# justinkay/aldi

Measured on AMD Instinct MI355X. Metric: images/sec (student+teacher ALDI step), R50-FPN 1333x800, higher is better.
Workload: dtype bf16

## Files before the change

### aldi_amd/csrc/host.h

```cpp
#pragma once
#include "../../include/aldi_hip.h"

int aldi_set_error_msg(int code, const char* msg);

typedef uint16_t bf16_t;

#define ALDI_KNOBS(X) \
    X(igemm_xcd, 1) X(igemm_tile, 0) X(igemm_dbg, 0) X(igemm_bigtile_min, 1024) X(igemm_bigtile, 64) X(igemm_bigtile_k, 768) X(igemm_lintile_min, 768) \
    X(igemm_halo, 1) X(igemm_force, 0) X(igemm_k64_min, 1024) X(igemm_group, 1) X(igemm_narrow_k, 512) X(igemm_splitk_tile, 2) X(igemm_halo_f32, 0) \
    X(igemm_f32_tile64_max, 4096) X(igemm_direct, 15) X(igemm_lean, 1) X(igemm_halo64_mid, 0) X(igemm_ws, 1) X(igemm_ws_wgs, 512) X(igemm_ws_min, 40000) \
    X(wgrad_lean, 1) X(wgrad_big_min, 28) X(wgrad_big_slots, 256) X(wgrad_slots, 384) X(wgrad_xcd, 1) \
    X(igemm_halo_ilv, 1) X(igemm_halo_small, 0) X(igemm_halo96, 0) \
    X(wgrad_dma, 0) X(wgrad_dbg, 0) X(wgrad_group_slots, 0) X(wgrad_group_epi, 24) X(wgrad_db, 0) X(wgrad_ordered, 1) X(wgrad_big_group, 1) X(wgrad_big_epi, 12) \
    X(wgrad_big_group_min, 64) X(wgrad_lds_pad_kb, 0) X(wgrad_f32_tile128, 1) X(wgrad_dma64, 3) X(wgrad_ilv, 0) \
    X(msda_gather, 7) X(msda_gather_list, 1500) X(msda_bin, 1) X(msda_bin_list, 512) X(roialign_sep, 1) X(roialign_bwd_rows, 2) \
    X(colsum_blocks, 256) X(colsum_minrows, 16) X(colsum_nt, 1024) X(colsum_block_kb, 384) \
    X(stem_mfma, 1) X(stem_pool_wgs, 0) X(sab_blocks, 512) X(ln_bwd_blocks, 512) X(ln_bwd_blocks_narrow, 1024) X(rpn_topk_fused, 1) X(ema_blocks, 2048) X(nms_mask_tri, 1) X(match_wave, 1)

struct AldiTuning {
#define ALDI_KNOB_FIELD(name, dflt) int name;
    ALDI_KNOBS(ALDI_KNOB_FIELD)
#undef ALDI_KNOB_FIELD
};
AldiTuning& aldi_tuning();
void aldi_note_dispatch(const char* kernel);

static inline int cdiv(long a, long b) { return (int)((a + b - 1) / b); }
```

### aldi_amd/csrc/roi.hip

```cpp
#include "common.h"
#include "loss_rows.h"
#include "sortscan.h"
#include "nms.h"
#include <hip/amd_detail/amd_hip_unsafe_atomics.h>


namespace {

__global__ void roi_append_gt_kernel(const float4* __restrict__ props, const int* __restrict__ pcount, int P,
                                     const float4* __restrict__ gt, const int* __restrict__ gcount, int Gmax,
                                     float4* __restrict__ cand, int* __restrict__ ccount, int Pcap) {
    const int n = blockIdx.y;
    const int i = blockIdx.x * blockDim.x + threadIdx.x;
    const int pc = pcount[n], gc = gcount[n];
    if (i == 0) ccount[n] = pc + gc;
    if (i >= Pcap) return;
    float4 v = make_float4(0, 0, 0, 0);
    if (i < pc) v = props[(long)n * P + i];
    else if (i < pc + gc) v = gt[(long)n * Gmax + (i - pc)];
    cand[(long)n * Pcap + i] = v;
}

__global__ void roi_classes_kernel(const int* __restrict__ labels, const int* __restrict__ best_idx, const int* __restrict__ gt_classes,
                                   const int* __restrict__ gcount, int Gmax, int L, int K, int* __restrict__ cls) {
// ... 827 lines not shown
        }
    }
#pragma unroll
    for (int r = 0; r < 2; ++r) {
        const int py = py0 + r;
        if (py >= H || px0 + px >= W) continue;
        const long o = (((long)b * H + py) * W + px0 + px) * C + cg * 4;
        if constexpr (sizeof(GT) == 2) {
            bf16_t* G = reinterpret_cast<bf16_t*>(ft.g[l]) + o;
#pragma unroll
            for (int j = 0; j < 8; ++j) {
                uint2 v;
                v.x = pack2_bf16(acc[r][j].x, acc[r][j].y); v.y = pack2_bf16(acc[r][j].z, acc[r][j].w);
                *reinterpret_cast<uint2*>(G + j * 32) = v;
            }
        } else {
            float* G = ft.g[l] + o;
#pragma unroll
            for (int j = 0; j < 8; ++j) *reinterpret_cast<float4*>(G + j * 32) = acc[r][j];
        }
    }
}

__global__ __launch_bounds__(256) void box_loss_kernel(const float* __restrict__ pred, int Cp, int K, int R,
                                                       const float* __restrict__ rois, const int* __restrict__ cls, const float4* __restrict__ gtb,
                                                       float wx, float wy, float ww, float wh, float gs_cls, float gs_box,
                                                       float* __restrict__ grad, float* __restrict__ loss ) {
    __shared__ float red[16];
    const int r = blockIdx.x * blockDim.x + threadIdx.x;
    float l_cls = 0.f, l_box = 0.f;
    const float invR = 1.f / (float)max(R, 1);
    if (r < R)
        box_loss_row(pred + (long)r * Cp, K, cls[r], rois + (long)r * 5, gtb[r], wx, wy, ww, wh, invR, gs_cls, gs_box, grad ? grad + (long)r * Cp : nullptr,
                     l_cls, l_box);
    float s0 = block_sum(l_cls, red);
    float s1 = block_sum(l_box, red);
    if (threadIdx.x == 0) {
        if (s0 != 0.f) unsafeAtomicAdd(loss + 0, s0 * invR);
        if (s1 != 0.f) unsafeAtomicAdd(loss + 1, s1 * invR);
    }
}

constexpr int kMaxLossChunks = 8;
struct BoxLossChunk {
    int r0, r1, blk0;
    float gs_cls, gs_box;
// ... 209 lines not shown
    GatherGeom gg;
    gg.N = N;
    const int rows = dtype == ALDI_BF16 && aldi_tuning().roialign_bwd_rows != 1 ? 2 : 1;
    int off = 0;
    for (int l = 0; l < 4; ++l) {
        if (!ft.g[l]) return aldi_set_error_msg(ALDI_ERR_ARG, "roialign_backward: missing gradient map");
        gg.blk_off[l] = off;
        gg.segs[l] = cdiv(ft.W[l], kSeg);
        off += N * cdiv(ft.H[l], rows) * gg.segs[l];
    }
    gg.blk_off[4] = off;
    hipStream_t st = static_cast<hipStream_t>(stream);
    if (rows == 2 && grad_dtype == ALDI_BF16)
        hipLaunchKernelGGL((roialign_bwd_gather2_kernel<bf16_t>), dim3(off), dim3(256), 0, st, ft, gg, rois, R, P, (const bf16_t*)g_pooled, rois_sorted);
    else if (rows == 2)
        hipLaunchKernelGGL((roialign_bwd_gather2_kernel<float>), dim3(off), dim3(256), 0, st, ft, gg, rois, R, P, (const bf16_t*)g_pooled, rois_sorted);
    else if (dtype == ALDI_BF16 && grad_dtype == ALDI_BF16)
        hipLaunchKernelGGL((roialign_bwd_gather_kernel<bf16_t, bf16_t>), dim3(off), dim3(256), 0, st, ft, gg, rois, R, P, (const bf16_t*)g_pooled, rois_sorted);
    else if (dtype == ALDI_BF16)
        hipLaunchKernelGGL((roialign_bwd_gather_kernel<bf16_t, float>), dim3(off), dim3(256), 0, st, ft, gg, rois, R, P, (const bf16_t*)g_pooled, rois_sorted);
    else if (dtype == ALDI_F32)
        hipLaunchKernelGGL((roialign_bwd_gather_kernel<float, float>), dim3(off), dim3(256), 0, st, ft, gg, rois, R, P, (const float*)g_pooled, rois_sorted);
    else return aldi_set_error_msg(ALDI_ERR_ARG, "roialign_backward: bad dtype");
    ALDI_CHECK_LAUNCH();
    return ALDI_OK;
}

extern "C" int aldi_box_loss(const float* pred, int Cp, int K, int R, const float* rois, const int* cls, const float* gt_boxes,
                             const float* weights4, float grad_scale_cls, float grad_scale_box, float* grad, float* loss2, aldi_stream_t stream) {
    if (!pred || !rois || !cls || !gt_boxes || !loss2 || !weights4) return aldi_set_error_msg(ALDI_ERR_ARG, "box_loss: null pointer");
    if (R <= 0) return ALDI_OK;
    hipLaunchKernelGGL(box_loss_kernel, dim3(cdiv(R, 256)), dim3(256), 0, static_cast<hipStream_t>(stream), pred, Cp, K, R, rois, cls, (const float4*)gt_boxes,
                       weights4[0], weights4[1], weights4[2], weights4[3], grad_scale_cls, grad_scale_box, grad, loss2);
    ALDI_CHECK_LAUNCH();
    return ALDI_OK;
}

extern "C" int aldi_box_losses_fused(const float* pred, int Cp, int K, const float* rois, const int* cls, const float* gt_boxes, const float* weights4,
                                     const aldi_box_loss_chunk* chunks, int nchunks, float* grad, void* grad_lo, aldi_stream_t stream) {
    if (!pred || !rois || !cls || !gt_boxes || !weights4 || !chunks || !grad) return aldi_set_error_msg(ALDI_ERR_ARG, "box_losses_fused: null pointer");
    if (nchunks < 1 || nchunks > kMaxLossChunks || (Cp & 1)) return aldi_set_error_msg(ALDI_ERR_ARG, "box_losses_fused: 1 .. 8 chunks, even row length");
    BoxLossArgs A;
    A.n = 0;
    int blk = 0;
    for (int i = 0; i < nchunks; ++i) {
        const aldi_box_loss_chunk& q = chunks[i];
// ... 63 lines not shown
```

### aldi_amd/engine.py

```python
from __future__ import annotations

import contextlib
import dataclasses
import inspect
import math
import os
from collections import OrderedDict
from typing import Dict, List, Optional, Sequence, Tuple

import torch

from . import ops
from .arch import FC_DIM, FPN_C, NUM_ANCHORS, POOL, STAGE_BLOCKS, Packed, ParamLayout, pad_to

PIXEL_MEAN = (103.530, 116.280, 123.675)
PIXEL_STD = (1.0, 1.0, 1.0)
ANCHOR_SIZES = (32, 64, 128, 256, 512)
ANCHOR_RATIOS = (0.5, 1.0, 2.0)
STRIDES = (4, 8, 16, 32, 64)
GMAX = 128
RPN_BATCH, RPN_POS_FRAC = 256, 0.5
ROI_BATCH, ROI_POS_FRAC = 512, 0.25
RPN_PRE = (2000, 1000)
RPN_POST = (1000, 1000)
RPN_NMS = 0.7
ROI_WEIGHTS = (10.0, 10.0, 5.0, 5.0)
SCORE_THRESH, NMS_TEST, DETS = 0.05, 0.5, 100


_FAST_RANDPERM = None


def randperm_prefix(n: int, k: int) -> torch.Tensor:
    global _FAST_RANDPERM
    from . import _lib as L
# ... 299 lines not shown
    if code & 1:
        raise FloatingPointError(f"{who}: predicted boxes or scores contain Inf/NaN. Training has diverged.")
    if code & 2:
        raise RuntimeError(f"{who}: sparse RPN-head backward: more active pixels than (2 * BATCH_SIZE_PER_IMAGE + 4 * positives) per image; "
                           "the excess was dropped, gradients of this step are wrong -- or, from the detection post-processing: a row of class "
                           "scores contains Inf/NaN; the row was dropped")
    if code & 4:
        raise RuntimeError(f"{who}: detection post-processing: more than 8192 candidates above SCORE_THRESH_TEST in one image; the excess was dropped")
    if code & 8:
        raise RuntimeError(f"{who}: RPN top-k: the group barrier of `topk_fused_kernel` timed out (its workgroups were not co-resident); the candidates "
                           "of this step are wrong.  Set ALDI_RPN_TOPK_FUSED=0 for the five-launch path")
    if code:
        raise RuntimeError(f"{who}: device error word {code}")


class Ctx(dict):
    __getattr__ = dict.__getitem__
    __setattr__ = dict.__setitem__


class RCNN:
    p = D2Params()
    stats_sink = None

    def __init__(self, weights: Weights, num_classes: int, params: Optional[D2Params] = None):
        self.wts = weights
        if params is not None:
            self.p = params
        self.K = num_classes
        self.device, self.dtype = weights.device, weights.dtype
        self.Cp = weights.layout.t["box_pred"].rows
        self.Ch = weights.layout.t["rpn_head_out"].rows
        self._anchor_cache: Dict[tuple, tuple] = {}
        self._ws: Dict[str, torch.Tensor] = {}
        self.err = torch.zeros(1, dtype=torch.int32, device=self.device)
        torch.set_num_threads(1)
        idx = lambda n: int(n.rsplit(".", 1)[1])
        names = list(getattr(weights.layout, "t", {}))
        self.img_da_layers = sorted((n for n in names if n.startswith("img_align.model.")), key=idx)
        self.ins_da_layers = sorted((n for n in names if n.startswith("ins_align.model.")), key=idx)
        self.has_img_da, self.has_ins_da = bool(self.img_da_layers), bool(self.ins_da_layers)
        self.fused_stem = os.environ.get("ALDI_FUSED_STEM", "1") == "1"
        self.wgrad_tail_split = int(os.environ.get("ALDI_WGRAD_TAIL_SPLIT", "2"))
        self.group_wgrad = os.environ.get("ALDI_WGRAD_GROUP", "1") == "1"
        self.mask_bits = os.environ.get("ALDI_MASK_BITS", "1") == "1"
        self.mask_bits_inner = os.environ.get("ALDI_MASK_BITS_INNER", "1") == "1"
        self.level_groups = os.environ.get("ALDI_LEVEL_GROUPS", "1") == "1"
        self.fused_res2 = os.environ.get("ALDI_FUSED_RES2", "1") == "1"
        self.fused_res2_shortcut = os.environ.get("ALDI_FUSED_RES2_SHORTCUT", "1") == "1"
        self.fused_stage_entrance = os.environ.get("ALDI_FUSED_STAGE_ENTRANCE", "1") == "1"
        self._wg_queue: list = []
        self.sparse_rpn_backward = os.environ.get("ALDI_RPN_SPARSE_BWD", "1") == "1"
        spec = getattr(weights.layout, "img_da", None)
        self.img_da_level = ("p2", "p3", "p4", "p5", "p6").index(spec["layer"]) if spec else 0

    def stage_images(self, images: Sequence[torch.Tensor]):
        sizes = [(int(im.shape[1]), int(im.shape[2])) for im in images]
        Hs = pad_to(max(s[0] for s in sizes), 32)
        Ws = pad_to(max(s[1] for s in sizes), 32)
        N = len(images)
        if all(im.is_cuda for im in images):
            st = torch.zeros((N, 3, Hs, Ws), dtype=torch.uint8, device=self.device)
            for i, im in enumerate(images):
                st[i, :, : sizes[i][0], : sizes[i][1]] = im
        else:
            host = torch.zeros((N, 3, Hs, Ws), dtype=torch.uint8).pin_memory()
            for i, im in enumerate(images):
                host[i, :, : sizes[i][0], : sizes[i][1]] = im
            st = host.to(self.device, non_blocking=True)
        hw = torch.tensor(sizes, dtype=torch.int32).to(self.device)
        return st, sizes, hw

    def stage_gt(self, instances: Sequence[dict]):
        N = len(instances)
        gb = torch.zeros((N, GMAX, 4), dtype=torch.float32)
# ... 584 lines not shown
        else:
            scratch = torch.empty((N, GMAX), dtype=torch.int32, device=dev)
            ops.roi_prepare(props, prop_count, P, gt["boxes"], gt["classes"], gt["count"], GMAX, N, self.K, self.p.roi_iou, cand, ccount, best_iou, best_idx,
                            scratch, labels, cls)
            ops.compact_labels(cls, Lc, N, self.K, lists, counts)
        return dict(cand=cand, cls=cls, best_idx=best_idx, lists=lists, counts=counts, Lc=Lc, counts_tail=cbuf)

    def _roi_gather(self, c: Ctx, prep: dict, sel, nsel, nsel_h, gt, N, row_off_dev=None):
        dev = self.device
        rows = [a + b for a, b in nsel_h]
        row_off = [0]
        for r in rows[:-1]:
            row_off.append(row_off[-1] + r)
        R = sum(rows)
        c.R, c.rows = R, rows
        c.rois = torch.empty((max(R, 1), 5), dtype=torch.float32, device=dev)
        c.r_cls = torch.empty((max(R, 1),), dtype=torch.int32, device=dev)
        c.r_gt = torch.empty((max(R, 1), 4), dtype=torch.float32, device=dev)
        c.r_idx = torch.empty((max(R, 1),), dtype=torch.int32, device=dev)
        if row_off_dev is None:
            row_off_dev = torch.tensor(row_off, dtype=torch.int32).to(dev)
        ops.roi_gather(prep["cand"], prep["cls"], prep["best_idx"], prep["Lc"], prep["lists"], sel, nsel, self.p.roi_batch,
                       row_off_dev, gt["boxes"], gt["count"], GMAX, N, c.rois, c.r_cls, c.r_gt, c.r_idx)

    def roi_sample(self, c: Ctx, props, prop_count, gt, N):
        prep = self._roi_prepare(props, prop_count, gt, N)
        host_counts = prep["counts"].cpu().tolist()
        c.roi_host_counts = host_counts
        sel, nsel, nsel_h = self._sample(host_counts, self.p.roi_batch, self.p.roi_pos_frac)
        self._roi_gather(c, prep, sel, nsel, nsel_h, gt, N)

    def roi_forward(self, c: Ctx):
        R = c.R
        pooled = torch.empty((R, POOL, POOL, FPN_C), dtype=self.dtype, device=self.device)
        ops.roialign(self.roi_feats(c), c.rois, R, POOL, pooled, backward=False)
        c.pred, _ = self.box_head(pooled, c)

    def box_head_on(self, c_feats: Ctx, rois: torch.Tensor, R: int):
        pooled = torch.empty((R, POOL, POOL, FPN_C), dtype=self.dtype, device=self.device)
        ops.roialign(self.roi_feats(c_feats), rois, R, POOL, pooled, backward=False)
        pred, fc2 = self.box_head(pooled)
        return pred

    def inference(self, images, pl_thresh: float, keep_ctx: bool = True, staged=None, pl_out=None) -> Ctx:
        st, sizes, hw = staged if staged is not None else self.stage_images(images)
        c = self.trunk(st, sizes, save=False)
# ... 83 lines not shown
            g_extra = None
            for al in align_list:
                if "ins" not in al:
                    continue
                acts, g_ = al["ins"]
                r0, r1 = al["r0"], al["r1"]
                if g_extra is None:
                    g_extra = torch.zeros((c.R, 1, 1, FC_DIM), dtype=T, device=dev)
                L_ = self.ins_da_layers
                for i in range(len(L_) - 1, -1, -1):
                    self._wgrad(L_[i], acts[i], g_)
                    if i == 0:
                        ops.conv2d(g_, W.wt(L_[0], negate=True), out=g_extra[r0:r1])
                    else:
                        g_ = ops.conv2d(g_, W.wt(L_[i]), mask=acts[i])
            lo = c.get("gpred_lo")
            gpred = (lo if lo is not None else ops.cast_from_f32(c.gpred[:c.R], T)).view(c.R, 1, 1, self.Cp)
            self._wgrad("box_pred", c.fc2, gpred)
            g_fc2 = ops.conv2d(gpred, W.wt("box_pred"), res=g_extra, res_mode=1 if g_extra is not None else 0, **self._relu_mask(c, c.fc2))
            self._wgrad("roi_heads.box_head.fc2", c.fc1, g_fc2)
            g_fc1 = ops.conv2d(g_fc2, W.wt("roi_heads.box_head.fc2"), mask=c.fc1)
            x = c.pooled.view(c.R, 1, 1, POOL * POOL * FPN_C)
            self._wgrad("roi_heads.box_head.fc1", x, g_fc1)
            g_pooled = ops.conv2d(g_fc1, W.wt("roi_heads.box_head.fc1")).view(c.R, POOL, POOL, FPN_C)
            ops.roialign_backward(self.roi_feats(c, gP_roi), c.rois, c.R, POOL, g_pooled, c.N, rois_sorted=True, grad_dtype=g_dt)
        self._grads_final(["box_pred", "roi_heads.box_head.fc2", "roi_heads.box_head.fc1"])
        if self.sparse_rpn_backward:
            if sp_pre is not None:
                main_ = torch.cuda.current_stream()
                main_.wait_stream(aux)
                for t_ in sp_pre.values():
                    if isinstance(t_, torch.Tensor):
                        t_.record_stream(main_)
                gP = self._rpn_sparse_finish(c, gP_roi, sp_pre)
            else:
                gP = self._rpn_head_backward_sparse(c, gP_roi)
        else:
            gP = []
            for l in range(5):
                gh = ops.cast_from_f32(c.ghead[l], T)
                self._wgrad("rpn_head_out", c.rpn_t[l], gh)
                g_t = ops.conv2d(gh, W.wt("rpn_head_out"), mask=c.rpn_t[l])
                self._wgrad("proposal_generator.rpn_head.conv", c.P[l], g_t)
                gP.append(ops.conv2d(g_t, W.wt("proposal_generator.rpn_head.conv"), pad=1))
            for l in range(4):
                ops.add_f32(gP[l], gP_roi[l], gP[l])
        for al in align_list:
            if "img" not in al:
# ... 136 lines not shown
        idx = torch.empty(cap, dtype=torch.int32, device=dev)
        count = torch.empty(1, dtype=torch.int32, device=dev)
        ws = torch.empty(ops.rpn_active_pixels_workspace(c.geom, N), dtype=torch.uint8, device=dev)
        ops.rpn_active_pixels(c.geom, c.ghead, N, cap, idx, count, ws, self.err)
        G = torch.empty((cap, 1, 1, Ch), dtype=T, device=dev)
        Tm = torch.empty((cap, 1, 1, Cf), dtype=T, device=dev)
        X9 = torch.empty((cap, 1, 1, 9 * Cf), dtype=T, device=dev)
        ops.rpn_sparse_gather(c.geom, c.ghead, c.rpn_t, c.P, N, Cf, cap, idx, count, G, Tm, X9)
        g_t = ops.conv2d(G, W.wt("rpn_head_out"), mask=Tm)
        Y = ops.conv2d(g_t, W.wt_flat("proposal_generator.rpn_head.conv"))
        return dict(cap=cap, idx=idx, count=count, G=G, Tm=Tm, X9=X9, g_t=g_t, Y=Y)

    def _rpn_sparse_finish(self, c: Ctx, gP_roi: List[torch.Tensor], sp: dict) -> List[torch.Tensor]:
        T, dev = self.dtype, self.device
        self._wgrad("rpn_head_out", sp["Tm"], sp["G"], temp_x=True)
        self._wgrad("proposal_generator.rpn_head.conv", sp["X9"], sp["g_t"], flat=True, temp_x=True)
        g32 = list(gP_roi) + [torch.zeros(c.P[4].shape, dtype=gP_roi[0].dtype, device=dev)]
        ops.rpn_sparse_scatter(c.geom, g32, sp["Y"], c.N, FPN_C, sp["cap"], sp["idx"], sp["count"])
        return g32 if g32[0].dtype == T else [ops.cast_from_f32(g, T) for g in g32]

    def _rpn_head_backward_sparse(self, c: Ctx, gP_roi: List[torch.Tensor]) -> List[torch.Tensor]:
        return self._rpn_sparse_finish(c, gP_roi, self._rpn_sparse_prepare(c))

    def _aux_stream(self):
        if not hasattr(self, "_aux_side"):
            self._aux_side = torch.cuda.Stream(device=self.device) if os.environ.get("ALDI_AUX_STREAM", "1") == "1" and torch.device(self.device).type == "cuda" else None
        return self._aux_side

    def _grads_final(self, names: List[str]):
        self._flush_wgrads()
        cb = getattr(self, "grad_ready", None)
        if cb is None:
            return
        evs = []
        side = getattr(self, "_wg_side", None)
        if side is not None and self._wgrad_pending:
            ev = torch.cuda.Event()
            ev.record(side)
            evs.append(ev)
        ev = torch.cuda.Event()
        ev.record()
        evs.append(ev)
        if len(inspect.signature(cb).parameters) >= 2:
            cb(self.wts.layout.ranges(names), evs)
        else:
            self._join_wgrads()
# ... 86 lines not shown
```

### aldi_amd/ops.py

```python
from __future__ import annotations

import ctypes as C
import os
from typing import List, NamedTuple, Optional, Sequence, Tuple

import torch

from . import _lib as L


def dtype_code(t: torch.dtype) -> int:
    if t == torch.float32:
        return L.F32
    if t == torch.bfloat16:
        return L.BF16
    raise TypeError(f"unsupported dtype {t}")


def _p(t: Optional[torch.Tensor]):
    return None if t is None else t.data_ptr()


_RAW_STREAM = getattr(torch._C, "_cuda_getCurrentRawStream", None)


def stream_ptr() -> int:
    if _RAW_STREAM is not None:
        return _RAW_STREAM(torch.cuda.current_device())
    return torch.cuda.current_stream().cuda_stream


# ... 527 lines not shown
    L.call("aldi_roi_prepare", _p(props), _p(pcount), P, _p(gt_boxes), _p(gt_classes), _p(gt_count), Gmax, N, K, thr, _p(cand), _p(ccount),
           _p(best_iou), _p(best_idx), _p(scratch), _p(labels), _p(cls), stream_ptr())


def roi_prepare_lists(props, pcount, P, gt_boxes, gt_classes, gt_count, Gmax, N, K, thr, cand, ccount, best_iou, best_idx, labels, cls, lists, counts, tickets,
                      tail_a=None, tail_b=None):
    L.call("aldi_roi_prepare_lists", _p(props), _p(pcount), P, _p(gt_boxes), _p(gt_classes), _p(gt_count), Gmax, N, K, thr, _p(cand), _p(ccount),
           _p(best_iou), _p(best_idx), _p(labels), _p(cls), _p(lists), _p(counts), _p(tickets), _p(tail_a), _p(tail_b), stream_ptr())


def roi_gather(cand, cls, best_idx, Lb, lists, sel, nsel, S, row_off, gt_boxes, gt_count, Gmax, N, rois, r_cls, r_gt, r_idx):
    L.call("aldi_roi_gather", _p(cand), _p(cls), _p(best_idx), Lb, _p(lists), _p(sel), _p(nsel), S, _p(row_off), _p(gt_boxes), _p(gt_count),
           Gmax, N, _p(rois), _p(r_cls), _p(r_gt), _p(r_idx), stream_ptr())


def rois_from_proposals(props, pcount, P, N, rois):
    L.call("aldi_rois_from_proposals", _p(props), _p(pcount), P, N, _p(rois), stream_ptr())


def roialign(feats: L.RoiFeats, rois, R, P, pooled, backward: bool):
    L.call("aldi_roialign", C.byref(feats), _p(rois), R, P, _p(pooled), int(backward), dtype_code(pooled.dtype), stream_ptr())


def roialign_backward(feats: L.RoiFeats, rois, R, P, g_pooled, N, rois_sorted: bool = False, grad_dtype=torch.float32):
    L.call("aldi_roialign_backward", C.byref(feats), _p(rois), R, P, _p(g_pooled), N, int(rois_sorted), dtype_code(g_pooled.dtype),
           dtype_code(grad_dtype), stream_ptr())


def box_loss(pred, Cp, K, R, rois, cls, gt_boxes, weights4, gs_cls, gs_box, grad, loss2):
    w = (C.c_float * 4)(*weights4)
    L.call("aldi_box_loss", _p(pred), Cp, K, R, _p(rois), _p(cls), _p(gt_boxes), w, gs_cls, gs_box, _p(grad), _p(loss2), stream_ptr())


def detections_workspace(N) -> int:
    return int(L.lib.aldi_detections_workspace(N))


def detections(pred, Cp, K, props, pcount, P, N, img_hw, weights4, score_thresh, nms_thresh, topk, pl_thresh, workspace,
               det_boxes, det_scores, det_cls, det_count, pl_boxes, pl_cls, pl_scores, pl_count, err):
    w = (C.c_float * 4)(*weights4)
    L.call("aldi_detections", _p(pred), Cp, K, _p(props), _p(pcount), P, N, _p(img_hw), w, score_thresh, nms_thresh, topk, pl_thresh,
           _p(workspace), _p(det_boxes), _p(det_scores), _p(det_cls), _p(det_count), _p(pl_boxes), _p(pl_cls), _p(pl_scores), _p(pl_count),
           pl_boxes.shape[1], _p(err), stream_ptr())


def rpn_distill_loss(geom, s_head, t_head, grad, labels, N, obj_T, n_valid, n_fg, do_obj, do_reg, grad_scale, loss2, counts_dev=None):
    L.call("aldi_rpn_distill_loss", C.byref(geom), ptrs(s_head), ptrs(t_head), ptrs(grad), _p(labels), N, obj_T, int(n_valid), int(n_fg),
# ... 125 lines not shown
```

### include/aldi_hip.h

```cpp
#ifndef ALDI_HIP_H
#define ALDI_HIP_H
#include <stddef.h>
#include <stdint.h>

#ifdef __cplusplus
extern "C" {
#endif

typedef void* aldi_stream_t;

enum { ALDI_F32 = 0, ALDI_BF16 = 1 };
enum { ALDI_OK = 0, ALDI_ERR_HIP = -1, ALDI_ERR_ARG = -2 };

const char* aldi_last_error(void);
int aldi_version(void);
int aldi_noop(aldi_stream_t stream);

int aldi_set_tuning(const char* name, int value);
int aldi_get_tuning(const char* name, int* value);
int aldi_reset_tuning(void);
const char* aldi_last_dispatch(void);

typedef struct {
    const void* x;
// ... 161 lines not shown
                            const int* count, int dtype, int grad_dtype, aldi_stream_t stream);

typedef struct {
    const void* feat[4];
    float* grad[4];
    int H[4], W[4];
    float scale[4];
    int C;
} aldi_roi_feats;

int aldi_roi_prepare(const float* props, const int* pcount, int P, const float* gt_boxes, const int* gt_classes, const int* gt_count,
                     int Gmax, int N, int K, float iou_thresh, float* cand, int* ccount, float* best_iou, int* best_idx,
                     unsigned* gt_best_scratch, int* labels, int* cls, aldi_stream_t stream);
int aldi_roi_prepare_lists(const float* props, const int* pcount, int P, const float* gt_boxes, const int* gt_classes, const int* gt_count,
                           int Gmax, int N, int K, float iou_thresh, float* cand, int* ccount, float* best_iou, int* best_idx, int* labels,
                           int* cls, int* lists, int* counts, unsigned* tickets, const int* tail_a, const int* tail_b, aldi_stream_t stream);
int aldi_roi_gather(const float* cand, const int* cls, const int* best_idx, int L, const int* lists, const int* sel, const int* nsel, int S,
                    const int* row_off, const float* gt_boxes, const int* gt_count, int Gmax, int N,
                    float* rois, int* r_cls, float* r_gt, int* r_idx, aldi_stream_t stream);
int aldi_rois_from_proposals(const float* props, const int* pcount, int P, int N, float* rois, aldi_stream_t stream);
int aldi_roialign(const aldi_roi_feats* f, const float* rois, int R, int P, void* pooled, int backward, int dtype, aldi_stream_t stream);
int aldi_roialign_backward(const aldi_roi_feats* f, const float* rois, int R, int P, const void* g_pooled, int N, int rois_sorted, int dtype,
                           int grad_dtype, aldi_stream_t stream);

int aldi_box_loss(const float* pred, int Cp, int K, int R, const float* rois, const int* cls, const float* gt_boxes,
                  const float* weights4, float grad_scale_cls, float grad_scale_box, float* grad, float* loss2, aldi_stream_t stream);
typedef struct {
    int r0, r1;
    float grad_scale_cls, grad_scale_box;
    float* loss_box;
    const float* teacher_pred;
    float cls_temperature;
    int kl, do_cls, do_reg;
    float grad_scale_distill_cls, grad_scale_distill_reg;
    float* loss_distill;
} aldi_box_loss_chunk;
int aldi_box_losses_fused(const float* pred, int Cp, int K, const float* rois, const int* cls, const float* gt_boxes, const float* weights4,
                          const aldi_box_loss_chunk* chunks, int nchunks, float* grad, void* grad_lo, aldi_stream_t stream);
size_t aldi_detections_workspace(int N);
int aldi_detections(const float* pred, int Cp, int K, const float* props, const int* pcount, int P, int N, const int* img_hw,
                    const float* weights4, float score_thresh, float nms_thresh, int topk, float pl_thresh, void* workspace,
                    float* det_boxes, float* det_scores, int* det_cls, int* det_count,
                    float* pl_boxes, int* pl_cls, float* pl_scores, int* pl_count, int pl_rows, int* err_flag, aldi_stream_t stream);

int aldi_rpn_distill_loss(const aldi_rpn_geom* gm, float* const* student_head, float* const* teacher_head, float* const* grad,
                          const int* labels, int N, float obj_temperature, int n_valid, int n_fg, const int* n_valid_fg_dev,
// ... 171 lines not shown
```

Baseline: 513.0.

## Build per-tile RoI lists for RoIAlign backward and chunk it across a side stream

Adds a pre-pass that computes compact per-RoI records and, for each (level, image, row-pair, 32-column segment) tile, a list of the RoIs that overlap it. The backward gather kernel then walks only its tile's list instead of scanning or binary-searching all RoIs. The Python side can also split the backward by image chunks on a side stream so the fc1 gradient GEMM for later chunks overlaps the gather for earlier ones. This adds list-building kernels, atomics and extra workspace, a bf16-only path, and stream synchronisation overhead.

```diff
diff --git a/aldi_amd/csrc/host.h b/aldi_amd/csrc/host.h
--- a/aldi_amd/csrc/host.h
+++ b/aldi_amd/csrc/host.h
@@ -13,7 +13,7 @@
     X(igemm_halo_ilv, 1) X(igemm_halo_small, 0) X(igemm_halo96, 0) \
     X(wgrad_dma, 0) X(wgrad_dbg, 0) X(wgrad_group_slots, 0) X(wgrad_group_epi, 24) X(wgrad_db, 0) X(wgrad_ordered, 1) X(wgrad_big_group, 1) X(wgrad_big_epi, 12) \
     X(wgrad_big_group_min, 64) X(wgrad_lds_pad_kb, 0) X(wgrad_f32_tile128, 1) X(wgrad_dma64, 3) X(wgrad_ilv, 0) \
-    X(msda_gather, 7) X(msda_gather_list, 1500) X(msda_bin, 1) X(msda_bin_list, 512) X(roialign_sep, 1) X(roialign_bwd_rows, 2) \
+    X(msda_gather, 7) X(msda_gather_list, 1500) X(msda_bin, 1) X(msda_bin_list, 512) X(roialign_sep, 1) X(roialign_bwd_rows, 2) X(roialign_lists, 1) X(roialign_bwd_chunks, 1) \
     X(colsum_blocks, 256) X(colsum_minrows, 16) X(colsum_nt, 1024) X(colsum_block_kb, 384) \
     X(stem_mfma, 1) X(stem_pool_wgs, 0) X(sab_blocks, 512) X(ln_bwd_blocks, 512) X(ln_bwd_blocks_narrow, 1024) X(rpn_topk_fused, 1) X(ema_blocks, 2048) X(nms_mask_tri, 1) X(match_wave, 1)
 
diff --git a/aldi_amd/csrc/roi.hip b/aldi_amd/csrc/roi.hip
--- a/aldi_amd/csrc/roi.hip
+++ b/aldi_amd/csrc/roi.hip
@@ -873,6 +873,299 @@
     }
 }
 
+struct RoiRec {
+    float x1, y1, bw, bh;
+    float inv; int gwh, img, lvl;
+    int r0, r1, c0, c1;
+};
+struct ListGeom { int blk_off[5]; int full_off[4]; int segs[4]; int b0; };
+
+__global__ __launch_bounds__(256) void roialign_records_kernel(Feats ft, const float* __restrict__ rois, int R, int P, RoiRec* __restrict__ recs,
+                                                               int* __restrict__ meta) {
+    const int r = blockIdx.x * blockDim.x + threadIdx.x;
+    if (r == 0) meta[0] = 0;
+    if (r >= R) return;
+    const float* rp = rois + (long)r * 5;
+    const int l = roi_level(rp[1], rp[2], rp[3], rp[4]);
+    const int H = ft.H[l], W = ft.W[l];
+    const float sc = ft.scale[l];
+    const float x1 = rp[1] * sc - 0.5f, y1 = rp[2] * sc - 0.5f;
+    const float x2 = rp[3] * sc - 0.5f, y2 = rp[4] * sc - 0.5f;
+    const float rw = x2 - x1, rh = y2 - y1;
+    const int r0 = min(max((int)floorf(y1) - 1, 0), H - 1), r1 = min(max((int)floorf(y2) + 2, 0), H - 1);
+    const int c0 = min(max((int)floorf(x1) - 1, 0), W - 1), c1 = min(max((int)floorf(x2) + 2, 0), W - 1);
+    const int gh = (int)ceilf(rh / (float)P), gw = (int)ceilf(rw / (float)P);
+    RoiRec o;
+    o.x1 = x1; o.y1 = y1; o.bw = rw / (float)P; o.bh = rh / (float)P;
+    o.inv = 1.f / (float)max(gh * gw, 1);
+    o.gwh = max(gw, 0) | (max(gh, 0) << 16);
+    o.img = (int)rp[0]; o.lvl = l;
+    o.r0 = r0; o.r1 = r1; o.c0 = c0; o.c1 = c1;
+    recs[r] = o;
+}
+
+constexpr int kMaxSegs = 64;
+struct PairGeom { int pair_off[5]; };
+__global__ __launch_bounds__(256) void roialign_lists_kernel(Feats ft, ListGeom lg, PairGeom pg, const RoiRec* __restrict__ recs, int R, int sorted,
+                                                             int nkeys, int* __restrict__ meta, int* __restrict__ idx) {
+    __shared__ int range[2];
+    __shared__ int cnt[kMaxSegs], start[kMaxSegs], wcnt[4][kMaxSegs];
+    const int tid = threadIdx.x, lane = tid & 63, wave = tid >> 6;
+    int l = 0;
+    while (l < 3 && (int)blockIdx.x >= pg.pair_off[l + 1]) ++l;
+    const int HP = (ft.H[l] + 1) >> 1, segs = lg.segs[l];
+    const int t = (int)blockIdx.x - pg.pair_off[l];
+    const int py0 = (t % HP) * 2, b = t / HP;
+    const int key0 = lg.blk_off[l] + t * segs;
+    int r_lo = 0, r_hi = R;
+    if (sorted && tid < 2) {
+        const int keyb = b + tid;
+        int lo = 0, hi = R;
+        while (lo < hi) {
+            const int mid = (lo + hi) >> 1;
+            if (recs[mid].img < keyb) lo = mid + 1; else hi = mid;
+        }
+        range[tid] = lo;
+    }
+    for (int s = tid; s < segs; s += 256) cnt[s] = 0;
+    __syncthreads();
+    if (sorted) { r_lo = range[0]; r_hi = range[1]; }
+    auto span = [&](int r, int& s0, int& s1) {
+        if (r >= r_hi) return false;
+        const RoiRec& c = recs[r];
+        if (!(c.img == b && c.lvl == l && py0 + 1 >= c.r0 && py0 <= c.r1)) return false;
+        s0 = c.c0 >> 5; s1 = min(c.c1 >> 5, segs - 1);
+        return s0 <= s1;
+    };
+    for (int base = r_lo; base < r_hi; base += 256) {
+        int s0 = 0, s1 = -1;
+        if (span(base + tid, s0, s1))
+            for (int s = s0; s <= s1; ++s) atomicAdd(&cnt[s], 1);
+    }
+    __syncthreads();
+    for (int s = tid; s < segs; s += 256) {
+        const int n = cnt[s];
+        const int st = n > 0 ? atomicAdd(meta, n) : 0;
+        meta[1 + key0 + s] = n;
+        meta[1 + nkeys + key0 + s] = st;
+        start[s] = st;
+    }
+    __syncthreads();
+    for (int base = r_lo; base < r_hi; base += 256) {
+        int s0 = 0, s1 = -1;
+        const bool h = span(base + tid, s0, s1);
+        for (int s = 0; s < segs; ++s) {
+            const unsigned long long m = __ballot(h && s0 <= s && s <= s1);
+            if (lane == 0) wcnt[wave][s] = __popcll(m);
+        }
+        __syncthreads();
+        for (int s = 0; s < segs; ++s) {
+            const bool hs = h && s0 <= s && s <= s1;
+            const unsigned long long m = __ballot(hs);
+            if (hs) {
+                int pos = start[s] + __popcll(m & ((1ull << lane) - 1ull));
+                for (int w = 0; w < wave; ++w) pos += wcnt[w][s];
+                idx[pos] = base + tid;
+            }
+        }
+        __syncthreads();
+        for (int s = tid; s < segs; s += 256) start[s] += wcnt[0][s] + wcnt[1][s] + wcnt[2][s] + wcnt[3][s];
+        __syncthreads();
+    }
+}
+
+template <typename GT>
+__global__ __launch_bounds__(256, 3) void roialign_bwd_gather2_lists_kernel(Feats ft, ListGeom lg, const RoiRec* __restrict__ recs, int nkeys,
+                                                                         const int* __restrict__ meta, const int* __restrict__ idx, int P,
+                                                                         const bf16_t* __restrict__ gp ) {
+    __shared__ int cand[256];
+    __shared__ float cx1[256], cy1[256], cbw[256], cbh[256], cinv[256];
+    __shared__ int cgwh[256];
+    __shared__ int rrun[4];
+    __shared__ __attribute__((aligned(16))) float rowc[4][2][8];
+    __shared__ __attribute__((aligned(16))) float colc[4][kSeg][8];
+    __shared__ __attribute__((aligned(16))) float gsum[2][2][7][256];
+    const int tid = threadIdx.x;
+    const int px = tid >> 3, cg = tid & 7;
+    const int qw = tid >> 5, c8 = tid & 31;
+    const int bid = (int)(gridDim.x - 1 - blockIdx.x);
+    int l = 0;
+    while (l < 3 && bid >= lg.blk_off[l + 1]) ++l;
+    const int H = ft.H[l], W = ft.W[l], C = ft.C;
+    const int HP = (H + 1) >> 1;
+    int t = bid - lg.blk_off[l];
+    const int seg = t % lg.segs[l]; t /= lg.segs[l];
+    const int py0 = (t % HP) * 2, b = lg.b0 + t / HP;
+    const int px0 = seg * kSeg;
+    const int key = lg.full_off[l] + (b * HP + (py0 >> 1)) * lg.segs[l] + seg;
+    const int nlist = __builtin_amdgcn_readfirstlane(meta[1 + key]);
+    const int* list = idx + __builtin_amdgcn_readfirstlane(meta[1 + nkeys + key]);
+    float4 acc[2][8];
+#pragma unroll
+    for (int r = 0; r < 2; ++r)
+#pragma unroll
+        for (int j = 0; j < 8; ++j) acc[r][j] = make_float4(0.f, 0.f, 0.f, 0.f);
+
+    auto tables = [&](int k, int buf) {
+        const float x1 = cx1[k], y1 = cy1[k], bw = cbw[k], bh = cbh[k];
+        const int gw = cgwh[k] & 0xffff, gh = cgwh[k] >> 16;
+        if (tid < 64) {
+            const int r = tid >> 3, ph = tid & 7, py = py0 + r;
+            float a = 0.f;
+            if (tid < 16 && ph < P && py < H)
+                for (int iy = 0; iy < gh; ++iy) {
+                    const Bilin by = bilin_prep(y1 + (float)ph * bh + ((float)iy + 0.5f) * bh / (float)gh, H);
+                    if (by.dead) continue;
+                    if (by.lo == py) a += by.h;
+                    if (by.hi == py) a += by.l;
+                }
+            const unsigned long long m = __ballot(a != 0.f);
+            if (tid < 16) rowc[buf][r][ph] = a;
+            if (tid == 0) {
+                const unsigned m0 = (unsigned)m & 0x7fu, m1 = (unsigned)(m >> 8) & 0x7fu, mm = m0 | m1;
+                rrun[buf] = mm ? (__ffs((int)mm) - 1) | ((31 - __clz((int)mm)) << 4) | ((m0 != 0) << 8) | ((m1 != 0) << 9) : 0;
+            }
+        }
+        {
+            const int pw = tid & 7;
+            float a = 0.f;
+            if (pw < P) {
+                const int pxa = px0 + px;
+                for (int ix = 0; ix < gw; ++ix) {
+                    const Bilin bx = bilin_prep(x1 + (float)pw * bw + ((float)ix + 0.5f) * bw / (float)gw, W);
+                    if (bx.dead) continue;
+                    if (bx.lo == pxa) a += bx.h;
+                    if (bx.hi == pxa) a += bx.l;
+                }
+            }
+            colc[buf][px][pw] = a;
+        }
+    };
+
+    for (int base = 0; base < nlist; base += 256) {
+        const int ncand = min(nlist - base, 256);
+        if (tid < ncand) {
+            const int r = list[base + tid];
+            const float4* rp = reinterpret_cast<const float4*>(recs + r);
+            const float4 g0 = rp[0], g1 = rp[1];
+            cand[tid] = r;
+            cx1[tid] = g0.x; cy1[tid] = g0.y; cbw[tid] = g0.z; cbh[tid] = g0.w;
+            cinv[tid] = g1.x; cgwh[tid] = __float_as_int(g1.y);
+        }
+        __syncthreads();
+        tables(0, 0);
+        if (ncand > 1) tables(1, 1);
+        __syncthreads();
+
+        uint4 raw[4];
+        float rc0[4] = {0.f, 0.f, 0.f, 0.f}, rc1[4] = {0.f, 0.f, 0.f, 0.f};
+        int plo = 0, phi = -1, lv = 0;
+        auto issue = [&](int k, int buf) {
+            const int m = rrun[buf];
+            lv = (m >> 8) & 3;
+            plo = m & 15; phi = lv ? (m >> 4) & 15 : -1;
+            if (!lv) return;
+            const bf16_t* g0 = gp + (long)cand[k] * P * P * C + c8 * 8;
+#pragma unroll
+            for (int j = 0; j < 4; ++j) {
+                const int ph = plo + j;
+                raw[j] = make_uint4(0u, 0u, 0u, 0u);
+                rc0[j] = 0.f; rc1[j] = 0.f;
+                if (ph <= phi) {
+                    rc0[j] = rowc[buf][0][ph]; rc1[j] = rowc[buf][1][ph];
+                    if (qw < P) raw[j] = *reinterpret_cast<const uint4*>(g0 + (long)(ph * P + qw) * C);
+                }
+            }
+        };
+        issue(0, 0);
+        for (int q = 0; q <= ncand; ++q) {
+            if (q < ncand) {
+                if (lv && qw < P) {
+                    float g0[8], g1[8], u[8];
+#pragma unroll
+                    for (int i = 0; i < 8; ++i) { g0[i] = 0.f; g1[i] = 0.f; }
+#pragma unroll
+                    for (int j = 0; j < 4; ++j) {
+                        Raw8<bf16_t> x; x.v = raw[j];
+                        x.unpack(u);
+                        fma8(g0, rc0[j], u);
+                        fma8(g1, rc1[j], u);
+                    }
+                    if (phi - plo > 3) {
+                        const bf16_t* gq = gp + (long)cand[q] * P * P * C + c8 * 8;
+                        for (int ph = plo + 4; ph <= phi; ++ph) {
+                            const float w0 = rowc[q & 3][0][ph], w1 = rowc[q & 3][1][ph];
+                            Raw8<bf16_t> x;
+                            x.load(gq + (long)(ph * P + qw) * C);
+                            x.unpack(u);
+                            { fma8(g0, w0, u); fma8(g1, w1, u); }
+                        }
+                    }
+                    const float inv = cinv[q];
+                    if (lv & 1) {
+                        float* gd = &gsum[q & 1][0][qw][c8 * 8];
+                        *reinterpret_cast<float4*>(gd) = make_float4(g0[0] * inv, g0[1] * inv, g0[2] * inv, g0[3] * inv);
+                        *reinterpret_cast<float4*>(gd + 4) = make_float4(g0[4] * inv, g0[5] * inv, g0[6] * inv, g0[7] * inv);
+                    }
+                    if (lv & 2) {
+                        float* gd = &gsum[q & 1][1][qw][c8 * 8];
+                        *reinterpret_cast<float4*>(gd) = make_float4(g1[0] * inv, g1[1] * inv, g1[2] * inv, g1[3] * inv);
+                        *reinterpret_cast<float4*>(gd + 4) = make_float4(g1[4] * inv, g1[5] * inv, g1[6] * inv, g1[7] * inv);
+                    }
+                }
+                if (q + 1 < ncand) issue(q + 1, (q + 1) & 3);
+                if (q + 2 < ncand) tables(q + 2, (q + 2) & 3);
+            }
+            if (q > 0) {
+                const int tb = (q - 1) & 3;
+                const int lvp = (rrun[tb] >> 8) & 3;
+                if (lvp) {
+                    const float4 w0 = *reinterpret_cast<const float4*>(&colc[tb][px][0]);
+                    const float4 w1 = *reinterpret_cast<const float4*>(&colc[tb][px][4]);
+                    const float wv[7] = {w0.x, w0.y, w0.z, w0.w, w1.x, w1.y, w1.z};
+#pragma unroll
+                    for (int r = 0; r < 2; ++r) {
+                        if (!((lvp >> r) & 1)) continue;
+                        const float* gsb = &gsum[(q - 1) & 1][r][0][cg * 4];
+#pragma unroll
+                        for (int pw = 0; pw < 7; ++pw) {
+                            if (wv[pw] != 0.f) {
+                                const float w = wv[pw];
+#pragma unroll
+                                for (int j = 0; j < 8; ++j) {
+                                    const float4 g = *reinterpret_cast<const float4*>(gsb + pw * 256 + j * 32);
+                                    float4& a = acc[r][j];
+                                    a.x = __builtin_fmaf(w, g.x, a.x); a.y = __builtin_fmaf(w, g.y, a.y); a.z = __builtin_fmaf(w, g.z, a.z); a.w = __builtin_fmaf(w, g.w, a.w);
+                                }
+                            }
+                        }
+                    }
+                }
+            }
+            __syncthreads();
+        }
+    }
+#pragma unroll
+    for (int r = 0; r < 2; ++r) {
+        const int py = py0 + r;
+        if (py >= H || px0 + px >= W) continue;
+        const long o = (((long)b * H + py) * W + px0 + px) * C + cg * 4;
+        if constexpr (sizeof(GT) == 2) {
+            bf16_t* G = reinterpret_cast<bf16_t*>(ft.g[l]) + o;
+#pragma unroll
+            for (int j = 0; j < 8; ++j) {
+                uint2 v;
+                v.x = pack2_bf16(acc[r][j].x, acc[r][j].y); v.y = pack2_bf16(acc[r][j].z, acc[r][j].w);
+                *reinterpret_cast<uint2*>(G + j * 32) = v;
+            }
+        } else {
+            float* G = ft.g[l] + o;
+#pragma unroll
+            for (int j = 0; j < 8; ++j) *reinterpret_cast<float4*>(G + j * 32) = acc[r][j];
+        }
+    }
+}
+
 __global__ __launch_bounds__(256) void box_loss_kernel(const float* __restrict__ pred, int Cp, int K, int R,
                                                        const float* __restrict__ rois, const int* __restrict__ cls, const float4* __restrict__ gtb,
                                                        float wx, float wy, float ww, float wh, float gs_cls, float gs_box,
@@ -1128,6 +1421,71 @@
     else if (dtype == ALDI_F32)
         hipLaunchKernelGGL((roialign_bwd_gather_kernel<float, float>), dim3(off), dim3(256), 0, st, ft, gg, rois, R, P, (const float*)g_pooled, rois_sorted);
     else return aldi_set_error_msg(ALDI_ERR_ARG, "roialign_backward: bad dtype");
+    ALDI_CHECK_LAUNCH();
+    return ALDI_OK;
+}
+
+static int list_geom(const Feats& ft, int nb, int* blk_off , int* segs , long* per_roi) {
+    int off = 0;
+    long most = 0;
+    for (int l = 0; l < 4; ++l) {
+        blk_off[l] = off;
+        segs[l] = cdiv(ft.W[l], kSeg);
+        const long one = (long)cdiv(ft.H[l], 2) * segs[l];
+        most = one > most ? one : most;
+        off += nb * (int)one;
+    }
+    blk_off[4] = off;
+    if (per_roi) *per_roi = most;
+    return off;
+}
+
+extern "C" int aldi_roialign_lists_build(const aldi_roi_feats* f, const float* rois, int R, int P, int N, int rois_sorted, void* records, int* meta,
+                                         int* idx, long idx_capacity, aldi_stream_t stream) {
+    if (!f || !records || !meta || !idx || (R > 0 && !rois) || R < 0 || P < 1 || P > 7 || N < 1)
+        return aldi_set_error_msg(ALDI_ERR_ARG, "roialign_lists_build: bad args (P <= 7)");
+    Feats ft = make_feats(f, false);
+    ListGeom lg;
+    long per_roi = 0;
+    const int nkeys = list_geom(ft, N, lg.blk_off, lg.segs, &per_roi);
+    if (idx_capacity < (long)R * per_roi) return aldi_set_error_msg(ALDI_ERR_ARG, "roialign_lists_build: idx_capacity below R * max_l(ceil(H_l / 2) * ceil(W_l / 32))");
+    for (int l = 0; l < 4; ++l) lg.full_off[l] = lg.blk_off[l];
+    lg.b0 = 0;
+    hipStream_t st = static_cast<hipStream_t>(stream);
+    hipLaunchKernelGGL(roialign_records_kernel, dim3(R > 0 ? cdiv(R, 256) : 1), dim3(256), 0, st, ft, rois, R, P, (RoiRec*)records, meta);
+    PairGeom pg;
+    pg.pair_off[0] = 0;
+    for (int l = 0; l < 4; ++l) {
+        if (lg.segs[l] > kMaxSegs) return aldi_set_error_msg(ALDI_ERR_ARG, "roialign_lists_build: maps wider than 2048 pixels");
+        pg.pair_off[l + 1] = pg.pair_off[l] + N * cdiv(ft.H[l], 2);
+    }
+    hipLaunchKernelGGL(roialign_lists_kernel, dim3(pg.pair_off[4]), dim3(256), 0, st, ft, lg, pg, (const RoiRec*)records, R, rois_sorted, nkeys, meta, idx);
+    ALDI_CHECK_LAUNCH();
+    return ALDI_OK;
+}
+
+extern "C" int aldi_roialign_backward_lists(const aldi_roi_feats* f, int P, const void* g_pooled, int N, int b0, int b1, const void* records,
+                                            const int* meta, const int* idx, int grad_dtype, aldi_stream_t stream) {
+    if (!f || !g_pooled || !records || !meta || !idx || f->C != 256 || P < 1 || P > 7 || N < 1 || b0 < 0 || b1 > N || b0 > b1)
+        return aldi_set_error_msg(ALDI_ERR_ARG, "roialign_backward_lists: bad args (C must be 256, P <= 7, 0 <= b0 <= b1 <= N)");
+    if (grad_dtype != ALDI_F32 && grad_dtype != ALDI_BF16) return aldi_set_error_msg(ALDI_ERR_ARG, "roialign_backward_lists: bad grad_dtype");
+    if (b0 == b1) return ALDI_OK;
+    Feats ft = make_feats(f, true);
+    for (int l = 0; l < 4; ++l)
+        if (!ft.g[l]) return aldi_set_error_msg(ALDI_ERR_ARG, "roialign_backward_lists: missing gradient map");
+    ListGeom lg;
+    int full[5];
+    const int nkeys = list_geom(ft, N, full, lg.segs, nullptr);
+    const int grid = list_geom(ft, b1 - b0, lg.blk_off, lg.segs, nullptr);
+    for (int l = 0; l < 4; ++l) lg.full_off[l] = full[l];
+    lg.b0 = b0;
+    hipStream_t st = static_cast<hipStream_t>(stream);
+    if (grad_dtype == ALDI_BF16)
+        hipLaunchKernelGGL((roialign_bwd_gather2_lists_kernel<bf16_t>), dim3(grid), dim3(256), 0, st, ft, lg, (const RoiRec*)records, nkeys, meta, idx, P,
+                           (const bf16_t*)g_pooled);
+    else
+        hipLaunchKernelGGL((roialign_bwd_gather2_lists_kernel<float>), dim3(grid), dim3(256), 0, st, ft, lg, (const RoiRec*)records, nkeys, meta, idx, P,
+                           (const bf16_t*)g_pooled);
     ALDI_CHECK_LAUNCH();
     return ALDI_OK;
 }
diff --git a/aldi_amd/engine.py b/aldi_amd/engine.py
--- a/aldi_amd/engine.py
+++ b/aldi_amd/engine.py
@@ -10,7 +10,7 @@
 
 import torch
 
-from . import ops
+from . import ops, roi_lists
 from .arch import FC_DIM, FPN_C, NUM_ANCHORS, POOL, STAGE_BLOCKS, Packed, ParamLayout, pad_to
 
 PIXEL_MEAN = (103.530, 116.280, 123.675)
@@ -356,6 +356,7 @@
 class RCNN:
     p = D2Params()
     stats_sink = None
+    roialign_lists, roi_bwd_chunks = False, 1
 
     def __init__(self, weights: Weights, num_classes: int, params: Optional[D2Params] = None):
         self.wts = weights
@@ -385,6 +386,8 @@
         self.fused_stage_entrance = os.environ.get("ALDI_FUSED_STAGE_ENTRANCE", "1") == "1"
         self._wg_queue: list = []
         self.sparse_rpn_backward = os.environ.get("ALDI_RPN_SPARSE_BWD", "1") == "1"
+        self.roialign_lists = ops.L.get_tuning("roialign_lists") != 0
+        self.roi_bwd_chunks = ops.L.get_tuning("roialign_bwd_chunks")
         spec = getattr(weights.layout, "img_da", None)
         self.img_da_level = ("p2", "p3", "p4", "p5", "p6").index(spec["layer"]) if spec else 0
 
@@ -1015,6 +1018,25 @@
             row_off_dev = torch.tensor(row_off, dtype=torch.int32).to(dev)
         ops.roi_gather(prep["cand"], prep["cls"], prep["best_idx"], prep["Lc"], prep["lists"], sel, nsel, self.p.roi_batch,
                        row_off_dev, gt["boxes"], gt["count"], GMAX, N, c.rois, c.r_cls, c.r_gt, c.r_idx)
+        self._roi_lists_build(c, N)
+
+    def _roi_lists_build(self, c: Ctx, N: int):
+        c.roi_lists = None
+        if not (self.roialign_lists and self.dtype == torch.bfloat16 and c.R > 0 and ops.L.get_tuning("roialign_bwd_rows") != 1):
+            return
+        feats = self.roi_feats(c)
+        nkeys, cap = roi_lists.sizes([(f.shape[1], f.shape[2]) for f in c.P[:4]], N, c.R)
+        i32 = lambda name, n: self.workspace(name, 4 * n)[: 4 * n].view(torch.int32)
+        lists = ops.RoiLists(i32("roi_records", c.R * roi_lists.REC_WORDS), i32("roi_list_meta", 1 + 2 * nkeys), i32("roi_list_idx", cap), nkeys)
+        aux, ev = self._aux_stream(), None
+        if aux is not None:
+            aux.wait_stream(torch.cuda.current_stream())
+        with torch.cuda.stream(aux) if aux is not None else contextlib.nullcontext():
+            ops.roialign_lists_build(feats, c.rois, c.R, POOL, N, lists, rois_sorted=True)
+            if aux is not None:
+                ev = torch.cuda.Event()
+                ev.record(aux)
+        c.roi_lists = dict(lists=lists, ev=ev, N=N)
 
     def roi_sample(self, c: Ctx, props, prop_count, gt, N):
         prep = self._roi_prepare(props, prop_count, gt, N)
@@ -1144,8 +1166,10 @@
             g_fc1 = ops.conv2d(g_fc2, W.wt("roi_heads.box_head.fc2"), mask=c.fc1)
             x = c.pooled.view(c.R, 1, 1, POOL * POOL * FPN_C)
             self._wgrad("roi_heads.box_head.fc1", x, g_fc1)
-            g_pooled = ops.conv2d(g_fc1, W.wt("roi_heads.box_head.fc1")).view(c.R, POOL, POOL, FPN_C)
-            ops.roialign_backward(self.roi_feats(c, gP_roi), c.rois, c.R, POOL, g_pooled, c.N, rois_sorted=True, grad_dtype=g_dt)
+            rl = c.get("roi_lists") if (self.roialign_lists and T == torch.bfloat16) else None
+            if rl is not None and rl["N"] != c.N:
+                rl = None
+            self._roi_backward(c, g_fc1, gP_roi, g_dt, rl)
         self._grads_final(["box_pred", "roi_heads.box_head.fc2", "roi_heads.box_head.fc1"])
         if self.sparse_rpn_backward:
             if sp_pre is not None:
@@ -1328,6 +1352,35 @@
     def _rpn_head_backward_sparse(self, c: Ctx, gP_roi: List[torch.Tensor]) -> List[torch.Tensor]:
         return self._rpn_sparse_finish(c, gP_roi, self._rpn_sparse_prepare(c))
 
+    def _roi_backward(self, c: Ctx, g_fc1, gP_roi, g_dt, rl):
+        W = self.wts
+        wt = W.wt("roi_heads.box_head.fc1")
+        lists = rl["lists"] if rl is not None else None
+        main = torch.cuda.current_stream()
+        if lists is not None and rl["ev"] is not None:
+            main.wait_event(rl["ev"])
+        side = self._roi_stream() if (lists is not None and self.roi_bwd_chunks > 1) else None
+        bounds = ops.roi_lists.image_chunks(c.rows, self.roi_bwd_chunks) if side is not None else []
+        if len(bounds) < 2:
+            g_pooled = ops.conv2d(g_fc1, wt).view(c.R, POOL, POOL, FPN_C)
+            ops.roialign_backward(self.roi_feats(c, gP_roi), c.rois, c.R, POOL, g_pooled, c.N, rois_sorted=True, grad_dtype=g_dt, lists=lists)
+            return
+        g_flat = torch.empty((c.R, 1, 1, POOL * POOL * FPN_C), dtype=g_fc1.dtype, device=self.device)
+        g_pooled = g_flat.view(c.R, POOL, POOL, FPN_C)
+        feats = self.roi_feats(c, gP_roi)
+        for b0, b1, r0, r1 in bounds:
+            if r1 > r0:
+                ops.conv2d(g_fc1[r0:r1], wt, out=g_flat[r0:r1])
+            side.wait_stream(main)
+            with torch.cuda.stream(side):
+                ops.roialign_backward(feats, c.rois, c.R, POOL, g_pooled, c.N, rois_sorted=True, grad_dtype=g_dt, lists=lists, images=(b0, b1))
+        main.wait_stream(side)
+
+    def _roi_stream(self):
+        if not hasattr(self, "_roi_side"):
+            self._roi_side = torch.cuda.Stream(device=self.device) if os.environ.get("ALDI_AUX_STREAM", "1") == "1" and torch.device(self.device).type == "cuda" else None
+        return self._roi_side
+
     def _aux_stream(self):
         if not hasattr(self, "_aux_side"):
             self._aux_side = torch.cuda.Stream(device=self.device) if os.environ.get("ALDI_AUX_STREAM", "1") == "1" and torch.device(self.device).type == "cuda" else None
diff --git a/aldi_amd/ops.py b/aldi_amd/ops.py
--- a/aldi_amd/ops.py
+++ b/aldi_amd/ops.py
@@ -7,6 +7,7 @@
 import torch
 
 from . import _lib as L
+from . import roi_lists
 
 
 def dtype_code(t: torch.dtype) -> int:
@@ -580,7 +581,35 @@
     L.call("aldi_roialign", C.byref(feats), _p(rois), R, P, _p(pooled), int(backward), dtype_code(pooled.dtype), stream_ptr())
 
 
-def roialign_backward(feats: L.RoiFeats, rois, R, P, g_pooled, N, rois_sorted: bool = False, grad_dtype=torch.float32):
+class RoiLists(NamedTuple):
+    records: torch.Tensor
+    meta: torch.Tensor
+    idx: torch.Tensor
+    nkeys: int
+
+
+def roialign_lists_alloc(feats: L.RoiFeats, R: int, N: int, device) -> RoiLists:
+    nkeys, cap = roi_lists.sizes([(feats.H[l], feats.W[l]) for l in range(4)], N, R)
+    return RoiLists(torch.empty((max(R, 1), roi_lists.REC_WORDS), dtype=torch.int32, device=device),
+                    torch.empty(1 + 2 * nkeys, dtype=torch.int32, device=device), torch.empty(max(cap, 1), dtype=torch.int32, device=device), nkeys)
+
+
+def roialign_lists_build(feats: L.RoiFeats, rois, R, P, N, lists: RoiLists, rois_sorted: bool = False):
+    L.call("aldi_roialign_lists_build", C.byref(feats), _p(rois), R, P, N, int(rois_sorted), _p(lists.records), _p(lists.meta), _p(lists.idx),
+           lists.idx.numel(), stream_ptr())
+
+
+def roialign_backward(feats: L.RoiFeats, rois, R, P, g_pooled, N, rois_sorted: bool = False, grad_dtype=torch.float32, lists: Optional[RoiLists] = None,
+                      images: Optional[Tuple[int, int]] = None):
+    if lists is not None:
+        if g_pooled.dtype != torch.bfloat16:
+            raise TypeError("roialign_backward: the list-driven gather takes bf16 pooled gradients")
+        b0, b1 = images if images is not None else (0, N)
+        L.call("aldi_roialign_backward_lists", C.byref(feats), P, _p(g_pooled), N, b0, b1, _p(lists.records), _p(lists.meta), _p(lists.idx),
+               dtype_code(grad_dtype), stream_ptr())
+        return
+    if images is not None:
+        raise ValueError("roialign_backward: an image range needs lists")
     L.call("aldi_roialign_backward", C.byref(feats), _p(rois), R, P, _p(g_pooled), N, int(rois_sorted), dtype_code(g_pooled.dtype),
            dtype_code(grad_dtype), stream_ptr())
 
diff --git a/aldi_amd/roi_lists.py b/aldi_amd/roi_lists.py
--- /dev/null
+++ b/aldi_amd/roi_lists.py
@@ -0,0 +1,68 @@
+from __future__ import annotations
+
+from typing import List, Sequence, Tuple
+
+SEG = 32
+REC_WORDS = 12
+
+
+def _cdiv(a: int, b: int) -> int:
+    return (a + b - 1) // b
+
+
+def per_image(shapes: Sequence[Tuple[int, int]]) -> List[int]:
+    return [_cdiv(h, 2) * _cdiv(w, SEG) for h, w in shapes]
+
+
+def key_offsets(shapes: Sequence[Tuple[int, int]], N: int) -> List[int]:
+    off = [0]
+    for n in per_image(shapes):
+        off.append(off[-1] + N * n)
+    return off
+
+
+def sizes(shapes: Sequence[Tuple[int, int]], N: int, R: int) -> Tuple[int, int]:
+    return key_offsets(shapes, N)[-1], R * max(per_image(shapes))
+
+
+def key_of(shapes: Sequence[Tuple[int, int]], N: int, level: int, image: int, pair: int, seg: int) -> int:
+    h, w = shapes[level]
+    return key_offsets(shapes, N)[level] + (image * _cdiv(h, 2) + pair) * _cdiv(w, SEG) + seg
+
+
+def reference_lists(records: Sequence[Sequence[int]], shapes: Sequence[Tuple[int, int]], N: int) -> List[List[int]]:
+    off = key_offsets(shapes, N)
+    out: List[List[int]] = [[] for _ in range(off[-1])]
+    for r, (img, lvl, r0, r1, c0, c1) in enumerate(records):
+        if not 0 <= img < N:
+            continue
+        h, w = shapes[lvl]
+        hp, segs = _cdiv(h, 2), _cdiv(w, SEG)
+        for pair in range(max(r0 // 2, 0), min(r1 // 2, hp - 1) + 1):
+            for seg in range(max(c0 // SEG, 0), min(c1 // SEG, segs - 1) + 1):
+                out[off[lvl] + (img * hp + pair) * segs + seg].append(r)
+    return out
+
+
+def brute_force_lists(records: Sequence[Sequence[int]], shapes: Sequence[Tuple[int, int]], N: int) -> List[List[int]]:
+    off = key_offsets(shapes, N)
+    out: List[List[int]] = [[] for _ in range(off[-1])]
+    for lvl, (h, w) in enumerate(shapes):
+        hp, segs = _cdiv(h, 2), _cdiv(w, SEG)
+        for img in range(N):
+            for pair in range(hp):
+                for seg in range(segs):
+                    py0, px0 = pair * 2, seg * SEG
+                    for r, (b, l, r0, r1, c0, c1) in enumerate(records):
+                        if b == img and l == lvl and py0 + 1 >= r0 and py0 <= r1 and c1 >= px0 and c0 < px0 + SEG:
+                            out[off[lvl] + (img * hp + pair) * segs + seg].append(r)
+    return out
+
+
+def image_chunks(rows: Sequence[int], chunks: int) -> List[Tuple[int, int, int, int]]:
+    n = len(rows)
+    per = _cdiv(n, max(min(chunks, n), 1)) if n else 1
+    off = [0]
+    for r in rows:
+        off.append(off[-1] + r)
+    return [(b, min(b + per, n), off[b], off[min(b + per, n)]) for b in range(0, n, per)]
diff --git a/include/aldi_hip.h b/include/aldi_hip.h
--- a/include/aldi_hip.h
+++ b/include/aldi_hip.h
@@ -207,6 +207,10 @@
 int aldi_roialign(const aldi_roi_feats* f, const float* rois, int R, int P, void* pooled, int backward, int dtype, aldi_stream_t stream);
 int aldi_roialign_backward(const aldi_roi_feats* f, const float* rois, int R, int P, const void* g_pooled, int N, int rois_sorted, int dtype,
                            int grad_dtype, aldi_stream_t stream);
+int aldi_roialign_lists_build(const aldi_roi_feats* f, const float* rois, int R, int P, int N, int rois_sorted, void* records, int* meta,
+                              int* idx, long idx_capacity, aldi_stream_t stream);
+int aldi_roialign_backward_lists(const aldi_roi_feats* f, int P, const void* g_pooled, int N, int b0, int b1, const void* records,
+                                 const int* meta, const int* idx, int grad_dtype, aldi_stream_t stream);
 
 int aldi_box_loss(const float* pred, int Cp, int K, int R, const float* rois, const int* cls, const float* gt_boxes,
                   const float* weights4, float grad_scale_cls, float grad_scale_box, float* grad, float* loss2, aldi_stream_t stream);
```

Result: no change. 510.3 (-0.5%).
